# fudan-zvg/tensoflow

Measured on NVIDIA B200. Metric: train rays/sec (fwd+bwd), higher is better.
Workload: dtype f32

## Files before the change

tensoflow_b200/csrc/mlp.cu:

```cuda
#include "common.cuh"
#include "act.cuh"

namespace {

constexpr int BM = 128, BN = 64, BK = 16, BMP = BM + 4, BNP = BN + 4;

template <bool TRANS_W, bool BWD>
__global__ void __launch_bounds__(256, 2) linear_kernel(const float* __restrict__ A, int lda, const float* __restrict__ Yact,
                                                        float* __restrict__ dpre, const float* __restrict__ W, int ldw,
                                                        const float* __restrict__ bias, int64_t M, int Kred, int Nout, int act,
                                                        float act_p, float* __restrict__ out, int ldo) {
    __shared__ __align__(16) float As[BK][BMP];
    __shared__ __align__(16) float Bs[BK][BNP];
    const int64_t r0 = (int64_t)blockIdx.x * BM;
    const int c0 = blockIdx.y * BN;
    const int ty = threadIdx.x / 16, tx = threadIdx.x % 16;
    float acc[8][4];
#pragma unroll
    for (int i = 0; i < 8; ++i) acc[i][0] = acc[i][1] = acc[i][2] = acc[i][3] = 0.f;
    for (int k0 = 0; k0 < Kred; k0 += BK) {
#pragma unroll
        for (int i = 0; i < BM / 16; ++i) {
            const int row = ty + 16 * i, k = tx;
            const int64_t r = r0 + row;
// ... 222 lines not shown
int tf_internal_xty(const float* X, int ldx, const float* Y, int ldy, int64_t rows, int M, int N, float* out, int ldo,
                    cudaStream_t stream) {
    if (rows == 0 || M == 0 || N == 0) return 0;
    dim3 grid((M + XT_M - 1) / XT_M, (N + XT_N - 1) / XT_N, 1);
    const int tiles = grid.x * grid.y;
    int64_t slices = (2 * (int64_t)tf_num_sms() + tiles - 1) / tiles;
    int64_t rpc = (rows + slices - 1) / slices;
    rpc = ((rpc + XT_R - 1) / XT_R) * XT_R;
    if (rpc < 256) rpc = 256;
    grid.z = (unsigned)((rows + rpc - 1) / rpc);
    xty_kernel<<<grid, 256, 0, stream>>>(X, ldx, Y, ldy, rows, M, N, out, ldo, rpc);
    tf_count_launches(1);
    return 0;
}

int tf_internal_matmul(const float* A, int lda, const float* W, int ldw, int64_t M, int Kred, int Nout, float* out, int ldo,
                       cudaStream_t stream) {
    if (M == 0 || Nout == 0) return 0;
    dim3 grid((unsigned)((M + BM - 1) / BM), (Nout + BN - 1) / BN);
    linear_kernel<true, false><<<grid, 256, 0, stream>>>(A, lda, nullptr, nullptr, W, ldw, nullptr, M, Kred, Nout, 0, 0.f, out, ldo);
    tf_count_launches(1);
    return 0;
}

int tf_internal_colsum(const float* X, int ldx, int64_t rows, int cols, float* out, cudaStream_t stream) {
    if (rows == 0 || cols == 0) return 0;
    int gy = (int)(rows < 1184 ? rows : 1184);
    dim3 cg((cols + 127) / 128, gy);
    colsum_kernel<<<cg, 128, 0, stream>>>(X, ldx, rows, cols, out);
    tf_count_launches(1);
    return 0;
}

constexpr int HEAD_NMAX = 8, HEAD_KMAX = 256;
bool head_shape(int64_t M, int K, int N, const void* a, const void* b) {
    return M >= 4096 && N <= HEAD_NMAX && K % 4 == 0 && K > SL_MAX && K <= HEAD_KMAX && (((uintptr_t)a | (uintptr_t)b) & 15) == 0;
}

template <int CH>
__global__ void __launch_bounds__(256) head_fwd_kernel(const float* __restrict__ X, const float* __restrict__ W, const float* __restrict__ b,
                                                       int64_t M, int K, int N, int act, float act_p, float* __restrict__ Y) {
    const int lane = threadIdx.x & 31, wpb = blockDim.x >> 5;
    float4 w[HEAD_NMAX][CH];
#pragma unroll
    for (int n = 0; n < HEAD_NMAX; ++n)
#pragma unroll
        for (int c = 0; c < CH; ++c) {
            const int k = c * 128 + lane * 4;
            w[n][c] = (n < N && k < K) ? *reinterpret_cast<const float4*>(W + (size_t)n * K + k) : f4_zero();
        }
    const float bias = (b && lane < N) ? b[lane] : 0.f;
    for (int64_t m = (int64_t)blockIdx.x * wpb + (threadIdx.x >> 5); m < M; m += (int64_t)gridDim.x * wpb) {
        float4 x[CH];
#pragma unroll
        for (int c = 0; c < CH; ++c) {
            const int k = c * 128 + lane * 4;
            x[c] = k < K ? ldg4(X + (size_t)m * K + k) : f4_zero();
        }
        float mine = 0.f;
#pragma unroll
        for (int n = 0; n < HEAD_NMAX; ++n) {
            if (n >= N) break;
            float a = 0.f;
#pragma unroll
            for (int c = 0; c < CH; ++c) a += (x[c].x * w[n][c].x + x[c].y * w[n][c].y) + (x[c].z * w[n][c].z + x[c].w * w[n][c].w);
#pragma unroll
            for (int o = 16; o > 0; o >>= 1) a += __shfl_xor_sync(0xffffffffu, a, o);
            if (lane == n) mine = a;
        }
        if (lane < N) Y[(size_t)m * N + lane] = act_fwd(mine + bias, act, act_p);
    }
}

template <int CH>
__global__ void __launch_bounds__(256) head_bwd_kernel(const float* __restrict__ X, const float* __restrict__ W, const float* __restrict__ Y,
                                                       const float* __restrict__ dY, int64_t M, int K, int N, int act, float act_p,
                                                       float* __restrict__ dX, float* __restrict__ dW, float* __restrict__ db) {
    __shared__ float red[8][HEAD_NMAX][HEAD_KMAX / 2 + 4];
    const int lane = threadIdx.x & 31, warp = threadIdx.x >> 5, wpb = blockDim.x >> 5;
    float4 w[HEAD_NMAX][CH], acc[HEAD_NMAX][CH];
#pragma unroll
    for (int n = 0; n < HEAD_NMAX; ++n)
#pragma unroll
        for (int c = 0; c < CH; ++c) {
            const int k = c * 128 + lane * 4;
            w[n][c] = (n < N && k < K) ? *reinterpret_cast<const float4*>(W + (size_t)n * K + k) : f4_zero();
            acc[n][c] = f4_zero();
        }
    float accb = 0.f;
    for (int64_t m = (int64_t)blockIdx.x * wpb + warp; m < M; m += (int64_t)gridDim.x * wpb) {
        float dp = 0.f;
        if (lane < N) { const size_t o = (size_t)m * N + lane; dp = __ldg(dY + o) * act_bwd(__ldg(Y + o), act, act_p); }
        accb += dp;
        float4 x[CH], dx[CH];
#pragma unroll
        for (int c = 0; c < CH; ++c) {
            const int k = c * 128 + lane * 4;
            x[c] = k < K ? ldg4(X + (size_t)m * K + k) : f4_zero();
            dx[c] = f4_zero();
        }
#pragma unroll
        for (int n = 0; n < HEAD_NMAX; ++n) {
            if (n >= N) break;
            const float d = __shfl_sync(0xffffffffu, dp, n);
#pragma unroll
            for (int c = 0; c < CH; ++c) { dx[c] = f4_fma(d, w[n][c], dx[c]); acc[n][c] = f4_fma(d, x[c], acc[n][c]); }
        }
        if (dX) {
#pragma unroll
            for (int c = 0; c < CH; ++c) {
                const int k = c * 128 + lane * 4;
                if (k < K) *reinterpret_cast<float4*>(dX + (size_t)m * K + k) = dx[c];
            }
        }
    }
#pragma unroll
    for (int c = 0; c < CH; ++c) {
        __syncthreads();
#pragma unroll
        for (int n = 0; n < HEAD_NMAX; ++n) *reinterpret_cast<float4*>(&red[warp][n][lane * 4]) = acc[n][c];
        __syncthreads();
        for (int i = threadIdx.x; i < N * 128; i += blockDim.x) {
            const int n = i >> 7, kk = i & 127, k = c * 128 + kk;
            if (k >= K) continue;
            float sum = 0.f;
            for (int wv = 0; wv < wpb; ++wv) sum += red[wv][n][kk];
            if (dW && sum != 0.f) atomicAdd(dW + (size_t)n * K + k, sum);
        }
    }
    if (db) {
        __syncthreads();
        if (lane < N) red[warp][lane][0] = accb;
        __syncthreads();
        if (threadIdx.x < N) {
            float sum = 0.f;
            for (int wv = 0; wv < wpb; ++wv) sum += red[wv][threadIdx.x][0];
            if (sum != 0.f) atomicAdd(db + threadIdx.x, sum);
        }
    }
}

int head_grid(int64_t M) {
    const int64_t want = (M + 127) / 128, cap = (int64_t)tf_num_sms() * 4;
    return (int)(want < cap ? want : cap);
}

bool tf_internal_linear_tc_ok(const float* X, const float* Y, int K, int N, int act);
size_t tf_internal_linear_tc_ws_floats(int K, int N);
int tf_internal_linear_tc(const float* X, const float* W, int ldw, int trans, const float* bias, int64_t M, int K, int N, int act, float act_p,
                          float* Y, float* wtc, cudaStream_t stream);
int tf_internal_linear_tc_bwd(const float* dY, const float* Yact, float* dpre, const float* W, int64_t M, int K, int N, int act, float act_p,
                              float* dX, float* wtc, cudaStream_t stream);
bool tf_internal_xty_tc_ok(const float* X, const float* Y, int M, int N);
int tf_internal_xty_tc(const float* X, const float* Y, int64_t rows, int M, int N, float* out, int ldo, int n_valid, cudaStream_t stream);

static const int64_t TC_MIN_ROWS = 8192;
static bool tc_shape(int64_t M, int K, int N) { return M >= TC_MIN_ROWS && K >= 96 && N >= 96; }

extern "C" TF_API size_t tf_linear_workspace(int32_t K, int32_t N) {
    if (K < 1 || N < 1) return 0;
    const size_t a = tf_internal_linear_tc_ws_floats(K, N), b = tf_internal_linear_tc_ws_floats(N, K);
    return (a > b ? a : b) * sizeof(float);
}

extern "C" TF_API int tf_linear_fwd(const float* X, const float* W, const float* b, int64_t M, int32_t K, int32_t N, int32_t act,
                                    float act_param, float* Y, void* workspace, size_t ws_bytes, tf_stream_t stream) {
    if (M == 0) return 0;
    TF_REQUIRE(X && W && Y, "tf_linear_fwd: NULL pointer");
    TF_REQUIRE(K > 0 && N > 0 && act >= 0 && act <= 5, "tf_linear_fwd: bad K/N/act (%d,%d,%d)", K, N, act);
    if (head_shape(M, K, N, X, W)) {
        if (K <= 128) head_fwd_kernel<1><<<head_grid(M), 256, 0, (cudaStream_t)stream>>>(X, W, b, M, K, N, act, act_param, Y);
        else head_fwd_kernel<2><<<head_grid(M), 256, 0, (cudaStream_t)stream>>>(X, W, b, M, K, N, act, act_param, Y);
        tf_count_launches(1);
        TF_CHECK_LAUNCH("tf_linear_fwd (head)");
        return 0;
    }
    if (workspace && tc_shape(M, K, N) && tf_internal_linear_tc_ok(X, Y, K, N, act) && ((uintptr_t)workspace & 15) == 0 &&
        ws_bytes >= tf_internal_linear_tc_ws_floats(K, N) * sizeof(float)) {
        tf_internal_linear_tc(X, W, K, 0, b, M, K, N, act, act_param, Y, (float*)workspace, (cudaStream_t)stream);
        TF_CHECK_LAUNCH("tf_linear_fwd (tcgen05)");
        return 0;
    }
    dim3 grid((unsigned)((M + BM - 1) / BM), (N + BN - 1) / BN);
    linear_kernel<false, false><<<grid, 256, 0, (cudaStream_t)stream>>>(X, K, nullptr, nullptr, W, K, b, M, K, N, act, act_param, Y, N);
    tf_count_launches(1);
    TF_CHECK_LAUNCH("tf_linear_fwd");
    return 0;
}

extern "C" TF_API int tf_linear_bwd(const float* X, const float* W, const float* Y, const float* dY, float* dpre, int64_t M,
                                    int32_t K, int32_t N, int32_t act, float act_param, float* dX, float* dW, float* db,
                                    void* workspace, size_t ws_bytes, tf_stream_t stream_) {
    if (M == 0) return 0;
    TF_REQUIRE(X && W && Y && dY && dpre && dY != dpre, "tf_linear_bwd: NULL pointer (or dY aliases dpre)");
    TF_REQUIRE(K > 0 && N > 0 && act >= 0 && act <= 5, "tf_linear_bwd: bad K/N/act (%d,%d,%d)", K, N, act);
    cudaStream_t stream = (cudaStream_t)stream_;
    if (K <= SL_MAX && N <= SL_MAX && M >= 4096) {
        const size_t smem = sizeof(float) * ((size_t)SL_ROWS * SL_DS + (size_t)SL_ROWS * SL_XS + (size_t)SL_MAX * SL_XS);
        cudaFuncSetAttribute(small_linear_bwd_kernel, cudaFuncAttributeMaxDynamicSharedMemorySize, (int)smem);
        const int64_t ntiles = (M + SL_ROWS - 1) / SL_ROWS;
        const int grid = (int)(ntiles < 2 * tf_num_sms() ? ntiles : 2 * tf_num_sms());
        small_linear_bwd_kernel<<<grid, 256, smem, stream>>>(X, W, Y, dY, M, K, N, act, act_param, dX, dW, db);
        tf_count_launches(1);
        TF_CHECK_LAUNCH("tf_linear_bwd (narrow)");
        return 0;
    }
    if (head_shape(M, K, N, X, W) && (!dX || ((uintptr_t)dX & 15) == 0)) {
        if (K <= 128) head_bwd_kernel<1><<<head_grid(M), 256, 0, stream>>>(X, W, Y, dY, M, K, N, act, act_param, dX, dW, db);
        else head_bwd_kernel<2><<<head_grid(M), 256, 0, stream>>>(X, W, Y, dY, M, K, N, act, act_param, dX, dW, db);
        tf_count_launches(1);
        TF_CHECK_LAUNCH("tf_linear_bwd (head)");
        return 0;
    }
    if (dX && workspace && tc_shape(M, K, N) && tf_internal_linear_tc_ok(dY, dX, N, K, act) && ((uintptr_t)workspace & 15) == 0 &&
        ws_bytes >= tf_internal_linear_tc_ws_floats(N, K) * sizeof(float)) {
        tf_internal_linear_tc_bwd(dY, Y, dpre, W, M, K, N, act, act_param, dX, (float*)workspace, stream);
    } else if (dX) {
        dim3 grid((unsigned)((M + BM - 1) / BM), (K + BN - 1) / BN);
        linear_kernel<true, true><<<grid, 256, 0, stream>>>(dY, N, Y, dpre, W, K, nullptr, M, N, K, act, act_param, dX, K);
        tf_count_launches(1);
    } else {
        dim3 grid((unsigned)((M + BM - 1) / BM), 1);
        linear_kernel<true, true><<<grid, 256, 0, stream>>>(dY, N, Y, dpre, W, K, nullptr, M, N, 0, act, act_param, nullptr, K);
        tf_count_launches(1);
    }
    if (dW) {
        if (tc_shape(M, K, N) && K % 16 == 0 && tf_internal_xty_tc_ok(dpre, X, N, K)) tf_internal_xty_tc(dpre, X, M, N, K, dW, K, K, stream);
        else tf_internal_xty(dpre, N, X, K, M, N, K, dW, K, stream);
    }
    if (db) tf_internal_colsum(dpre, N, M, N, db, stream);
    TF_CHECK_LAUNCH("tf_linear_bwd");
    return 0;
}
```

tensoflow_b200/csrc/sdf_stencil.cu:

```cuda
#include <stdlib.h>
#include "common.cuh"

namespace {

constexpr int TS = 16;
constexpr int NQ = 7;
constexpr int R = TS * NQ;
constexpr int NC = 32;
constexpr int NT = 256;
constexpr int HCS = NC + 2;

__host__ __device__ inline int round_up4(int x) { return (x + 3) & ~3; }

__global__ void prep_weights_kernel(const float* __restrict__ W0, const float* __restrict__ W1, int K, int KP, int H, int A,
                                    float* __restrict__ W0T, float* __restrict__ W0P, float* __restrict__ W1T) {
    const int tid = blockIdx.x * blockDim.x + threadIdx.x, nth = gridDim.x * blockDim.x;
    for (int i = tid; i < KP * H; i += nth) {
        const int k = i / H, h = i % H;
        W0T[i] = k < K ? W0[h * K + k] : 0.f;
    }
    for (int i = tid; i < H * KP; i += nth) {
        const int h = i / KP, k = i % KP;
        W0P[i] = k < K ? W0[h * K + k] : 0.f;
    }
// ... 386 lines not shown
    TF_REQUIRE(m && m->W0 && m->b0 && m->W1 && m->b1, "MLP descriptor / weights are NULL");
    TF_REQUIRE(m->hidden > 0 && m->hidden % NC == 0, "hidden must be a multiple of %d (got %d)", NC, m->hidden);
    TF_REQUIRE(m->app_dim >= 4 && m->app_dim % 4 == 0 && m->app_dim <= 128, "app_dim must be a multiple of 4 in [4,128] (got %d)", m->app_dim);
    TF_REQUIRE(f->n_comp <= 36, "n_comp <= 36 supported by the fused stencil (got %d)", f->n_comp);
    d.C = f->n_comp; d.K = 3 * d.C + 3; d.KP = round_up4(d.K); d.KS = d.KP + 4; d.H = m->hidden; d.A = m->app_dim;
    return 0;
}

size_t weights_ws_floats(const Dims& d) { return (size_t)2 * d.KP * d.H + (size_t)d.H * d.A; }

size_t fwd_smem(const Dims& d, bool feat) {
    return sizeof(float) * ((size_t)R * d.KS + (size_t)d.KP * NC + (feat ? (size_t)NC * d.A + TS * HCS : 0));
}
size_t bwd_smem(const Dims& d) {
    return sizeof(float) * ((size_t)R * d.KS + (size_t)d.KP * NC + (size_t)NC * d.KS + (size_t)R * DSS + (size_t)TS * d.A +
                            (size_t)(1 + d.A) * NC + NQ * TS + 2 * d.H + 4);
}

void fill_common(StencilParams& p, const tf_vm_field_t* f, const tf_sdf_mlp_t* m, const Dims& d, const float* xyz,
                 const float* level, int64_t n, const float units[3], float* ws) {
    p.f = *f; p.xyz = xyz; p.level = level; p.n = n;
    p.W0T = ws; p.W0P = ws + (size_t)d.KP * d.H; p.W1T = ws + (size_t)2 * d.KP * d.H;
    p.b0 = m->b0; p.W1 = m->W1; p.b1 = m->b1;
    p.K = d.K; p.KP = d.KP; p.KS = d.KS; p.H = d.H; p.A = d.A;
    p.units[0] = units ? units[0] : 0.f; p.units[1] = units ? units[1] : 0.f; p.units[2] = units ? units[2] : 0.f;
}

}

int tf_check_field(const tf_vm_field_t* f, bool need_mips);

bool tf_internal_linear_tc_ok(const float* X, const float* Y, int K, int N, int act);
size_t tf_internal_linear_tc_ws_floats(int K, int N);
int tf_internal_linear_tc(const float* X, const float* W, int ldw, int trans, const float* bias, int64_t M, int K, int N, int act, float act_p,
                          float* Y, float* wtc, cudaStream_t stream);
size_t tf_internal_tc_fwd_smem(int KT, int H);
size_t tf_internal_tc_w0_floats(int KT, int H);
int tf_internal_stencil_fwd_tc(const tf_vm_field_t* f, const tf_sdf_mlp_t* m, const float* xyz, const float* level, int64_t n,
                               const float units[3], int nq, float* sdf7, float* grad, float* hess, float* sdf1, float* spc,
                               float* w0tc, cudaStream_t stream);
static bool use_simt_path(const Dims& d) {
    static int forced = -1;
    if (forced < 0) { const char* e = getenv("TF_STENCIL_SIMT"); forced = (e && e[0] == '1') ? 1 : 0; }
    const int KT = (d.K + 15) / 16 * 16;
    return forced == 1 || tf_internal_tc_fwd_smem(KT, d.H) > 227 * 1024 || KT > 128 || d.H > 256 || d.H % 32 != 0;
}

static size_t fwd_ws_floats(const Dims& d, int64_t n, bool with_feat) {
    if (use_simt_path(d)) return weights_ws_floats(d);
    const int KT = (d.K + 15) / 16 * 16;
    return tf_internal_tc_w0_floats(KT, d.H) + (with_feat ? (size_t)(n < 1 ? 1 : n) * d.H + tf_internal_linear_tc_ws_floats(d.H, d.A) : 0);
}

extern "C" TF_API size_t tf_sdf_stencil_fwd_workspace(const tf_vm_field_t* f, const tf_sdf_mlp_t* m, int64_t n, int32_t with_feat) {
    Dims d;
    if (!f || !m || check_mlp(f, m, d)) return 0;
    return fwd_ws_floats(d, n, with_feat != 0) * sizeof(float);
}

static int stencil_fwd_impl(int mode, const tf_vm_field_t* f, const tf_sdf_mlp_t* m, const float* xyz, const float* level,
                            int64_t n, const float units[3], float* sdf7, float* feat, float* grad, float* hess, float* sdf1,
                            void* workspace, size_t ws_bytes, tf_stream_t stream_) {
    if (int e = tf_check_field(f, level != nullptr)) return e;
    Dims d;
    if (int e = check_mlp(f, m, d)) return e;
    if (n == 0) return 0;
    TF_REQUIRE(xyz, "xyz is NULL");
    TF_REQUIRE(workspace && ws_bytes >= fwd_ws_floats(d, n, feat != nullptr) * sizeof(float), "workspace too small (%zu bytes)", ws_bytes);
    TF_REQUIRE(((uintptr_t)workspace & 15) == 0, "workspace not 16-byte aligned");
    if (feat) TF_REQUIRE(((uintptr_t)feat & 15) == 0, "feat not 16-byte aligned");
    cudaStream_t stream = (cudaStream_t)stream_;
    if (!use_simt_path(d)) {
        const int KT = (d.K + 15) / 16 * 16;
        float* w0tc = (float*)workspace;
        float* spc = feat ? w0tc + tf_internal_tc_w0_floats(KT, d.H) : nullptr;
        if (mode == 0) TF_REQUIRE(sdf7, "sdf7 is NULL"); else TF_REQUIRE(sdf1, "sdf is NULL");
        if (int e = tf_internal_stencil_fwd_tc(f, m, xyz, level, n, units, mode == 0 ? 7 : 1, sdf7, grad, hess, sdf1, spc, w0tc, stream)) return e;
        if (feat) {
            float* wlin = spc + (size_t)n * d.H;
            if (tf_internal_linear_tc_ok(spc, feat, d.H, d.A, 0))
                tf_internal_linear_tc(spc, m->W1 + d.H, d.H, 0, m->b1 + 1, n, d.H, d.A, 0, 0.f, feat, wlin, stream);
            else if (int e = tf_linear_fwd(spc, m->W1 + d.H, m->b1 + 1, n, d.H, d.A, 0, 0.f, feat, nullptr, 0, stream_)) return e;
        }
        TF_CHECK_LAUNCH("tf_sdf_stencil_fwd (tcgen05)");
        return 0;
    }
    StencilParams p = {};
    fill_common(p, f, m, d, xyz, level, n, units, (float*)workspace);
    p.sdf7 = sdf7; p.feat = feat; p.grad = grad; p.hess = hess; p.sdf1 = sdf1;
    prep_weights_kernel<<<64, 256, 0, stream>>>(m->W0, m->W1, d.K, d.KP, d.H, d.A, (float*)p.W0T, (float*)p.W0P, (float*)p.W1T);
    const int64_t per_tile = mode == 0 ? TS : R;
    const int64_t ntiles = (n + per_tile - 1) / per_tile;
    const int64_t cap = (int64_t)tf_num_sms() * 2;
    const int grid = (int)(ntiles < cap ? ntiles : cap);
    if (mode == 0) {
        TF_REQUIRE(sdf7, "sdf7 is NULL");
        const size_t smem = fwd_smem(d, feat != nullptr);
        cudaFuncSetAttribute(sdf_stencil_fwd_kernel<0>, cudaFuncAttributeMaxDynamicSharedMemorySize, (int)smem);
        sdf_stencil_fwd_kernel<0><<<grid, NT, smem, stream>>>(p);
    } else {
        TF_REQUIRE(sdf1, "sdf is NULL");
        const size_t smem = fwd_smem(d, false);
        cudaFuncSetAttribute(sdf_stencil_fwd_kernel<1>, cudaFuncAttributeMaxDynamicSharedMemorySize, (int)smem);
        sdf_stencil_fwd_kernel<1><<<grid, NT, smem, stream>>>(p);
    }
    tf_count_launches(2);
    TF_CHECK_LAUNCH("tf_sdf_stencil_fwd");
    return 0;
}

extern "C" TF_API int tf_sdf_stencil_fwd(const tf_vm_field_t* f, const tf_sdf_mlp_t* m, const float* xyz, const float* level,
                                  int64_t n, const float units[3], float* sdf7, float* feat, float* grad, float* hess,
                                  void* workspace, size_t ws_bytes, tf_stream_t stream) {
    TF_REQUIRE(units, "units is NULL");
    return stencil_fwd_impl(0, f, m, xyz, level, n, units, sdf7, feat, grad, hess, nullptr, workspace, ws_bytes, stream);
}

extern "C" TF_API int tf_sdf_only_fwd(const tf_vm_field_t* f, const tf_sdf_mlp_t* m, const float* xyz, const float* level, int64_t n,
                               float* sdf, void* workspace, size_t ws_bytes, tf_stream_t stream) {
    return stencil_fwd_impl(1, f, m, xyz, level, n, nullptr, nullptr, nullptr, nullptr, nullptr, sdf, workspace, ws_bytes, stream);
}

extern "C" TF_API int tf_sdf_point_fwd(const tf_vm_field_t* f, const tf_sdf_mlp_t* m, const float* xyz, const float* level, int64_t n,
                                       float* sdf, float* feat, void* workspace, size_t ws_bytes, tf_stream_t stream) {
    Dims d;
    if (!f || !m) { tf_set_error("tf_sdf_point_fwd: NULL descriptor"); return 1; }
    if (int e = check_mlp(f, m, d)) return e;
    TF_REQUIRE(feat, "tf_sdf_point_fwd: feat is NULL (use tf_sdf_only_fwd for the SDF alone)");
    TF_REQUIRE(!use_simt_path(d), "tf_sdf_point_fwd: only the tensor-core path evaluates single queries with features "
                                  "(hidden %% 32 == 0, hidden <= 256); use tf_sdf_stencil_fwd");
    return stencil_fwd_impl(1, f, m, xyz, level, n, nullptr, nullptr, feat, nullptr, nullptr, sdf, workspace, ws_bytes, stream);
}

static size_t bwd_slice_floats(const Dims& d, int64_t n_slice) {
    const int64_t tiles = (n_slice + TS - 1) / TS;
    return (size_t)tiles * ((size_t)R * d.H + (size_t)R * d.KP + (size_t)TS * d.H);
}

size_t tf_internal_bwd_tc_wtc_floats(int KT, int H);
size_t tf_internal_bwd_tc_smem(int KT, int H);
int tf_internal_bwd_tc_prep(const float* W0, int K, int KT, int H, float* wtc, cudaStream_t stream);
int tf_internal_bwd_tc_samples_per_tile();
int tf_internal_bwd_tc_fold(const float* tmp, int H, int K, int KT, float* dW0, float* db0, cudaStream_t stream);
int tf_internal_stencil_bwd_tc(const tf_vm_field_t* f, const tf_vm_mut_t* g, const tf_sdf_mlp_t* m, const float* wtc, const float* xyz,
                               const float* level, int64_t n, const float units[3], const float* sdf7, const float* g_sdf,
                               const float* g_grad, const float* g_hess, const float* dHc, float* dpre, float* arow, float* spc,
                               float* da_scratch, float* dW1r0, float* db1, cudaStream_t stream);
size_t tf_internal_bwd_tc_scratch_floats(int KT);
int tf_internal_xty(const float* X, int ldx, const float* Y, int ldy, int64_t rows, int M, int N, float* out, int ldo, cudaStream_t stream);
int tf_internal_colsum(const float* X, int ldx, int64_t rows, int cols, float* out, cudaStream_t stream);
int tf_internal_matmul(const float* A, int lda, const float* W, int ldw, int64_t M, int Kred, int Nout, float* out, int ldo,
                       cudaStream_t stream);
bool tf_internal_xty_tc_ok(const float* X, const float* Y, int M, int N);
int tf_internal_xty_tc(const float* X, const float* Y, int64_t rows, int M, int N, float* out, int ldo, int n_valid, cudaStream_t stream);
int tf_internal_xty_tc_tiled(const float* X, const float* Y, int64_t rows, int M, int N, float* out, int ldo, int n_valid, int x_tiled,
                             cudaStream_t stream);

static bool use_simt_bwd(const Dims& d) {
    const int KT = (d.K + 15) / 16 * 16;
    return use_simt_path(d) || d.C % 4 != 0 || KT > 128  || tf_internal_bwd_tc_smem(KT, d.H) > 227 * 1024;
}
static size_t bwd_tc_fixed_floats(const Dims& d) {
    const int KT = (d.K + 15) / 16 * 16;
    return tf_internal_bwd_tc_wtc_floats(KT, d.H) + (size_t)d.H * KT + tf_internal_linear_tc_ws_floats(d.A, d.H) +
           tf_internal_bwd_tc_scratch_floats(KT);
}
static size_t bwd_tc_tile_floats(const Dims& d) {
    const int KT = (d.K + 15) / 16 * 16, spt = tf_internal_bwd_tc_samples_per_tile();
    return (size_t)128 * (d.H + KT) + 2 * (size_t)spt * d.H;
}

extern "C" TF_API size_t tf_sdf_stencil_bwd_workspace(const tf_vm_field_t* f, const tf_sdf_mlp_t* m, int64_t n_slice) {
    Dims d;
    if (!f || !m || check_mlp(f, m, d)) return 0;
    if (n_slice < 1) n_slice = 1;
    if (!use_simt_bwd(d)) {
        const int spt = tf_internal_bwd_tc_samples_per_tile();
        return (bwd_tc_fixed_floats(d) + (size_t)((n_slice + spt - 1) / spt) * bwd_tc_tile_floats(d)) * sizeof(float);
    }
    return (weights_ws_floats(d) + bwd_slice_floats(d, n_slice)) * sizeof(float);
}

static int stencil_bwd_tc(const tf_vm_field_t* f, const tf_sdf_mlp_t* m, const Dims& d, const float* xyz, const float* level, int64_t n,
                          const float units[3], const float* sdf7, const float* g_sdf, const float* g_feat, const float* g_grad,
                          const float* g_hess, const tf_vm_mut_t* g_field, const tf_sdf_mlp_grad_t* g_mlp, float* ws, size_t ws_floats,
                          const float* hidden_c, cudaStream_t stream) {
    const int KT = (d.K + 15) / 16 * 16, H = d.H;
    const int spt = tf_internal_bwd_tc_samples_per_tile();
    const size_t fixed = bwd_tc_fixed_floats(d), per_tile = bwd_tc_tile_floats(d);
    TF_REQUIRE(ws_floats >= fixed + per_tile, "workspace too small (%zu bytes)", ws_floats * sizeof(float));
    int64_t tiles_fit = (int64_t)((ws_floats - fixed) / per_tile);
    const int64_t ntiles_all = (n + spt - 1) / spt;
    if (tiles_fit > ntiles_all) tiles_fit = ntiles_all;
    float* wtc = ws;
    float* tmp = wtc + tf_internal_bwd_tc_wtc_floats(KT, H);
    float* wlin = tmp + (size_t)H * KT;
    float* da_scratch = wlin + tf_internal_linear_tc_ws_floats(d.A, H);
    float* dpre = da_scratch + tf_internal_bwd_tc_scratch_floats(KT);
    float* arow = dpre + (size_t)tiles_fit * 128 * H;
    float* spc = arow + (size_t)tiles_fit * 128 * KT;
    float* dHc = spc + (size_t)tiles_fit * spt * H;
    tf_internal_bwd_tc_prep(m->W0, d.K, KT, H, wtc, stream);
    cudaMemsetAsync(tmp, 0, (size_t)H * KT * sizeof(float), stream);
    for (int64_t t0 = 0; t0 < ntiles_all; t0 += tiles_fit) {
        const int64_t nt = t0 + tiles_fit < ntiles_all ? tiles_fit : ntiles_all - t0;
        const int64_t s0 = t0 * spt;
        const int64_t ns = s0 + nt * spt < n ? nt * spt : n - s0;
        const float* gf = g_feat ? g_feat + s0 * d.A : nullptr;
        if (gf) {
            if (tf_internal_linear_tc_ok(gf, dHc, d.A, H, 0)) tf_internal_linear_tc(gf, m->W1 + H, H, 1, nullptr, ns, d.A, H, 0, 0.f, dHc, wlin, stream);
            else tf_internal_matmul(gf, d.A, m->W1 + H, H, ns, d.A, H, dHc, H, stream);
        }
        if (int e = tf_internal_stencil_bwd_tc(f, g_field, m, wtc, xyz + s0 * 3, level ? level + s0 : nullptr, ns, units, sdf7 + s0 * NQ,
                                               g_sdf ? g_sdf + s0 : nullptr, g_grad ? g_grad + s0 * 3 : nullptr,
                                               g_hess ? g_hess + s0 : nullptr, gf ? dHc : nullptr, dpre, arow, (gf && !hidden_c) ? spc : nullptr,
                                               da_scratch, g_mlp->W1, g_mlp->b1, stream))
            return e;
        TF_REQUIRE(tf_internal_xty_tc_ok(dpre, arow, H, KT), "tensor-core X^T Y does not take this decoder shape (H=%d, KT=%d)", H, KT);
        if (int e = tf_internal_xty_tc_tiled(dpre, arow, nt * 128, H, KT, tmp, KT, d.K + 1, 1, stream)) return e;
        if (gf) {
            const float* hid = hidden_c ? hidden_c + s0 * H : spc;
            if (tf_internal_xty_tc_ok(gf, hid, d.A, H)) tf_internal_xty_tc(gf, hid, ns, d.A, H, g_mlp->W1 + H, H, H, stream);
            else tf_internal_xty(gf, d.A, hid, H, ns, d.A, H, g_mlp->W1 + H, H, stream);
            tf_internal_colsum(gf, d.A, ns, d.A, g_mlp->b1 + 1, stream);
        }
    }
    tf_internal_bwd_tc_fold(tmp, H, d.K, KT, g_mlp->W0, g_mlp->b0, stream);
    TF_CHECK_LAUNCH("tf_sdf_stencil_bwd (tcgen05)");
    return 0;
}

extern "C" TF_API size_t tf_sdf_stencil_fwd_hidden_offset(const tf_vm_field_t* f, const tf_sdf_mlp_t* m) {
    Dims d;
    if (!f || !m || check_mlp(f, m, d) || use_simt_path(d)) return (size_t)-1;
    const int KT = (d.K + 15) / 16 * 16;
    return tf_internal_tc_w0_floats(KT, d.H) * sizeof(float);
}

extern "C" TF_API int tf_sdf_stencil_bwd(const tf_vm_field_t* f, const tf_sdf_mlp_t* m, const float* xyz, const float* level,
                                  int64_t n, const float units[3], const float* sdf7, const float* g_sdf, const float* g_feat,
                                  const float* g_grad, const float* g_hess, const tf_vm_mut_t* g_field,
                                  const tf_sdf_mlp_grad_t* g_mlp, void* workspace, size_t ws_bytes, tf_stream_t stream_) {
    return tf_sdf_stencil_bwd_kept(f, m, xyz, level, n, units, sdf7, nullptr, g_sdf, g_feat, g_grad, g_hess, g_field, g_mlp, workspace, ws_bytes,
                                   stream_);
}

extern "C" TF_API int tf_sdf_stencil_bwd_kept(const tf_vm_field_t* f, const tf_sdf_mlp_t* m, const float* xyz, const float* level,
                                       int64_t n, const float units[3], const float* sdf7, const float* hidden_centre, const float* g_sdf,
                                       const float* g_feat, const float* g_grad, const float* g_hess, const tf_vm_mut_t* g_field,
                                       const tf_sdf_mlp_grad_t* g_mlp, void* workspace, size_t ws_bytes, tf_stream_t stream_) {
    if (int e = tf_check_field(f, level != nullptr)) return e;
    Dims d;
    if (int e = check_mlp(f, m, d)) return e;
    if (n == 0) return 0;
    TF_REQUIRE(xyz && units && sdf7, "xyz/units/sdf7 is NULL");
    TF_REQUIRE(g_field && g_mlp && g_mlp->W0 && g_mlp->b0 && g_mlp->W1 && g_mlp->b1, "gradient descriptors are NULL");
    for (int i = 0; i < 3; ++i) {
        TF_REQUIRE(g_field->plane[i] && g_field->line[i], "gradient buffer %d is NULL", i);
        if (f->n_levels > 1 && level) TF_REQUIRE(g_field->plane_mip[i] && g_field->line_mip[i], "mip gradient buffer %d is NULL", i);
    }
    TF_REQUIRE(((uintptr_t)workspace & 15) == 0, "workspace not 16-byte aligned");
    if (g_feat) TF_REQUIRE(((uintptr_t)g_feat & 15) == 0, "g_feat not 16-byte aligned");
    cudaStream_t stream = (cudaStream_t)stream_;
    float* ws = (float*)workspace;
    TF_REQUIRE(workspace, "workspace is NULL");
    if (hidden_centre) TF_REQUIRE(((uintptr_t)hidden_centre & 15) == 0, "hidden_centre not 16-byte aligned");
    if (!use_simt_bwd(d))
        return stencil_bwd_tc(f, m, d, xyz, level, n, units, sdf7, g_sdf, g_feat, g_grad, g_hess, g_field, g_mlp, ws,
                              ws_bytes / sizeof(float), hidden_centre, stream);
    const size_t wfl = weights_ws_floats(d);
    TF_REQUIRE(ws_bytes >= (wfl + bwd_slice_floats(d, TS)) * sizeof(float), "workspace too small (%zu bytes)", ws_bytes);
    const size_t per_tile = (size_t)R * d.H + (size_t)R * d.KP + (size_t)TS * d.H;
    int64_t tiles_fit = (int64_t)((ws_bytes / sizeof(float) - wfl) / per_tile);
    const int64_t ntiles_all = (n + TS - 1) / TS;
    if (tiles_fit > ntiles_all) tiles_fit = ntiles_all;
    const size_t smem = bwd_smem(d);
    cudaFuncSetAttribute(sdf_stencil_bwd_kernel, cudaFuncAttributeMaxDynamicSharedMemorySize, (int)smem);
    StencilParams p = {};
    fill_common(p, f, m, d, xyz, level, n, units, ws);
    prep_weights_kernel<<<64, 256, 0, stream>>>(m->W0, m->W1, d.K, d.KP, d.H, d.A, (float*)p.W0T, (float*)p.W0P, (float*)p.W1T);
    tf_count_launches(1);
    float* dpre = ws + wfl;
    float* arow = dpre + (size_t)tiles_fit * R * d.H;
    float* spc = arow + (size_t)tiles_fit * R * d.KP;
    for (int64_t t0 = 0; t0 < ntiles_all; t0 += tiles_fit) {
        const int64_t nt = t0 + tiles_fit < ntiles_all ? tiles_fit : ntiles_all - t0;
        const int64_t s0 = t0 * TS;
        const int64_t ns = (s0 + nt * TS < n ? nt * TS : n - s0);
        StencilParams q = p;
        q.xyz = xyz + s0 * 3; q.level = level ? level + s0 : nullptr; q.n = ns;
        q.sdf7_in = sdf7 + s0 * NQ;
        q.g_sdf = g_sdf ? g_sdf + s0 : nullptr; q.g_feat = g_feat ? g_feat + s0 * d.A : nullptr;
        q.g_grad = g_grad ? g_grad + s0 * 3 : nullptr; q.g_hess = g_hess ? g_hess + s0 : nullptr;
        q.g = *g_field;
        q.dpre = dpre; q.arow = arow; q.spc = spc;
        q.db0 = g_mlp->b0; q.dW1r0 = g_mlp->W1; q.db1 = g_mlp->b1;
        const int64_t cap = tf_num_sms();
        const int grid = (int)(nt < cap ? nt : cap);
        sdf_stencil_bwd_kernel<<<grid, NT, smem, stream>>>(q);
        tf_count_launches(1);
        tf_internal_xty(dpre, d.H, arow, d.KP, nt * R, d.H, d.K, g_mlp->W0, d.K, stream);
        if (g_feat) {
            tf_internal_xty(q.g_feat, d.A, spc, d.H, ns, d.A, d.H, g_mlp->W1 + d.H, d.H, stream);
            tf_internal_colsum(q.g_feat, d.A, ns, d.A, g_mlp->b1 + 1, stream);
        }
    }
    TF_CHECK_LAUNCH("tf_sdf_stencil_bwd");
    return 0;
}
```

tensoflow_b200/csrc/xty_tc.cu:

```cuda
#include <stdlib.h>
#include "common.cuh"
#include "tc_common.cuh"

namespace {

constexpr int NTH = 512;
constexpr int NWORK = NTH - 32;
constexpr int TPT = 2;
constexpr uint32_t LBO = 144;
template <int RS> struct Stage { static constexpr uint32_t SBO = (RS / 4) * LBO + 16; };

__device__ __forceinline__ float4 hi4(float4 v) { return make_float4(tc::tf32_rn(v.x), tc::tf32_rn(v.y), tc::tf32_rn(v.z), tc::tf32_rn(v.w)); }
__device__ __forceinline__ float4 lo4(float4 v, float4 h) {
    return make_float4(tc::tf32_rn(v.x - h.x), tc::tf32_rn(v.y - h.y), tc::tf32_rn(v.z - h.z), tc::tf32_rn(v.w - h.w));
}

struct Prefetch { float4 v[TPT][4]; };
struct StagePlan { int src_off[TPT]; int row[TPT]; int ld[TPT]; uint32_t smem_off[TPT]; bool on[TPT], is_x[TPT], tiled[TPT]; };

template <int RS>
__device__ __forceinline__ StagePlan make_stage_plan(int M, int N, int wtid, bool x_tiled, bool y_tiled) {
    constexpr uint32_t SBO = Stage<RS>::SBO;
    StagePlan p;
    const int ty = (RS / 4) * (N / 4), tx = (RS / 4) * (M / 4);
#pragma unroll
    for (int k = 0; k < TPT; ++k) {
        int it = wtid + k * NWORK;
        p.is_x[k] = it >= ty;
        if (p.is_x[k]) it -= ty;
        const int W = p.is_x[k] ? M : N, G = W / 4;
        p.on[k] = wtid >= 0 && it < (p.is_x[k] ? tx : ty);
        p.tiled[k] = p.is_x[k] ? x_tiled : y_tiled;
        const int g = p.tiled[k] ? it / (RS / 4) : it % G, c = p.tiled[k] ? it % (RS / 4) : it / G;
        p.row[k] = c * 4;
        p.ld[k] = p.tiled[k] ? 128 : W;
        p.src_off[k] = p.tiled[k] ? g * 4 * 128 + c * 4 : c * 4 * W + g * 4;
        const int w = g * 4;
        p.smem_off[k] = (uint32_t)(w >> 3) * SBO + c * LBO + (w & 7) * 16;
    }
    return p;
}
__device__ __forceinline__ void stage_load(const float* __restrict__ X, const float* __restrict__ Y, int64_t r0, int64_t r_end, int M, int N,
                                           const StagePlan& sp, Prefetch& pf) {
#pragma unroll
    for (int k = 0; k < TPT; ++k) {
        if (sp.tiled[k]) {
            const float* base = (sp.is_x[k] ? X + (size_t)(r0 >> 7) * 128 * M : Y + (size_t)(r0 >> 7) * 128 * N) + (r0 & 127) + sp.src_off[k];
#pragma unroll
            for (int i = 0; i < 4; ++i) pf.v[k][i] = (sp.on[k] && r0 + sp.row[k] < r_end) ? ldg4(base + i * 128) : make_float4(0.f, 0.f, 0.f, 0.f);
        } else {
            const float* base = (sp.is_x[k] ? X : Y) + (size_t)r0 * sp.ld[k] + sp.src_off[k];
#pragma unroll
            for (int i = 0; i < 4; ++i)
                pf.v[k][i] = (sp.on[k] && r0 + sp.row[k] + i < r_end) ? ldg4(base + i * sp.ld[k]) : make_float4(0.f, 0.f, 0.f, 0.f);
        }
    }
}
__device__ __forceinline__ void stage_store(const Prefetch& pf, const StagePlan& sp, uint8_t* xs_hi, uint8_t* xs_lo, uint8_t* ys_hi, uint8_t* ys_lo) {
#pragma unroll
    for (int k = 0; k < TPT; ++k) {
        if (!sp.on[k]) continue;
        uint8_t* hi = sp.is_x[k] ? xs_hi : ys_hi;
        uint8_t* lo = sp.is_x[k] ? xs_lo : ys_lo;
        const float4* v = pf.v[k];
        float4 t[4];
        if (sp.tiled[k]) {
            t[0] = v[0]; t[1] = v[1]; t[2] = v[2]; t[3] = v[3];
        } else {
            t[0] = make_float4(v[0].x, v[1].x, v[2].x, v[3].x); t[1] = make_float4(v[0].y, v[1].y, v[2].y, v[3].y);
            t[2] = make_float4(v[0].z, v[1].z, v[2].z, v[3].z); t[3] = make_float4(v[0].w, v[1].w, v[2].w, v[3].w);
        }
#pragma unroll
        for (int j = 0; j < 4; ++j) {
            const uint32_t off = sp.smem_off[k] + j * 16;
            const float4 h = hi4(t[j]);
            *reinterpret_cast<float4*>(hi + off) = h;
            *reinterpret_cast<float4*>(lo + off) = lo4(t[j], h);
        }
    }
}

template <int RS>
__global__ void __launch_bounds__(NTH, 1) xty_tc_kernel(const float* __restrict__ X, const float* __restrict__ Y, int64_t rows, int M, int MP, int N,
                                                        float* __restrict__ out, int ldo, int x_valid, int y_valid, int tr, int64_t rows_per_cta,
                                                        int x_tiled, int y_tiled) {
    extern __shared__ __align__(1024) uint8_t smem[];
    constexpr uint32_t SBO = Stage<RS>::SBO;
    const uint32_t x_part = (uint32_t)(MP / 8) * SBO, y_part = (uint32_t)(N / 8) * SBO;
    const uint32_t stage_bytes = 2 * (x_part + y_part);
    uint64_t* bars = reinterpret_cast<uint64_t*>(smem + 2 * stage_bytes);
    uint64_t* empty = bars;
    uint64_t* ready = bars + 2;
    uint64_t* done = bars + 4;
    uint32_t* tmem_slot = reinterpret_cast<uint32_t*>(bars + 5);
    const int tid = threadIdx.x, warp = tid >> 5, lane = tid & 31;
    const int MT = MP / 128;
    const int ncol_tile = N <= 128 ? 128 : 256;

    if (warp == 0) tc::tmem_alloc<512>(tmem_slot);
    if (tid == 0) {
        tc::mbar_init(&empty[0], 1); tc::mbar_init(&empty[1], 1); tc::mbar_init(&ready[0], NWORK); tc::mbar_init(&ready[1], NWORK);
        tc::mbar_init(done, 1);
        tc::mbar_fence_init();
    }
    for (uint32_t i = tid * 16; i < 2 * stage_bytes; i += NTH * 16) *reinterpret_cast<float4*>(smem + i) = make_float4(0.f, 0.f, 0.f, 0.f);
    tc::fence_async_smem();
    tc::fence_before_sync();
    __syncthreads();
    tc::fence_after_sync();
    const uint32_t tmem_base = *tmem_slot;
    const uint32_t idesc = tc::make_idesc(2, 2, 128, N);

    const int64_t r_begin = (int64_t)blockIdx.x * rows_per_cta;
    const int64_t r_end = r_begin + rows_per_cta < rows ? r_begin + rows_per_cta : rows;
    const int64_t n_stages = r_begin < r_end ? (r_end - r_begin + RS - 1) / RS : 0;

    if (warp == 0) {
        if (lane == 0) {
            for (int64_t it = 0; it < n_stages; ++it) {
                const int buf = (int)(it & 1);
                uint8_t* xs_hi = smem + (size_t)buf * stage_bytes;
                uint8_t* xs_lo = xs_hi + x_part;
                uint8_t* ys_hi = xs_lo + x_part;
                uint8_t* ys_lo = ys_hi + y_part;
                tc::mbar_wait(&ready[buf], (uint32_t)((it >> 1) & 1));
                tc::fence_after_sync();
                const uint64_t xdh = tc::make_smem_desc(tc::smem_u32(xs_hi), LBO, SBO), xdl = tc::make_smem_desc(tc::smem_u32(xs_lo), LBO, SBO);
                const uint64_t ydh = tc::make_smem_desc(tc::smem_u32(ys_hi), LBO, SBO), ydl = tc::make_smem_desc(tc::smem_u32(ys_lo), LBO, SBO);
#pragma unroll
                for (int ks = 0; ks < RS / 8; ++ks) {
                    const uint64_t bdh = tc::desc_add(ydh, ks * 2 * LBO), bdl = tc::desc_add(ydl, ks * 2 * LBO);
#pragma unroll
                    for (int mt = 0; mt < 2; ++mt) {
                        if (mt >= MT) break;
                        const uint32_t d = tmem_base + (uint32_t)mt * ncol_tile;
                        const uint64_t adh = tc::desc_add(xdh, mt * 16 * SBO + ks * 2 * LBO), adl = tc::desc_add(xdl, mt * 16 * SBO + ks * 2 * LBO);
                        tc::mma_tf32_ss(d, adh, bdh, idesc, (it | ks) != 0);
                        tc::mma_tf32_ss(d, adh, bdl, idesc, 1);
                        tc::mma_tf32_ss(d, adl, bdh, idesc, 1);
                    }
                }
                tc::mma_commit(&empty[buf]);
                if (it == n_stages - 1) tc::mma_commit(done);
            }
        }
    } else {
        Prefetch p0, p1;
        const StagePlan sp = make_stage_plan<RS>(M, N, tid - 32, x_tiled != 0, y_tiled != 0);
        if (n_stages > 0) stage_load(X, Y, r_begin, r_end, M, N, sp, p0);
        if (n_stages > 1) stage_load(X, Y, r_begin + RS, r_end, M, N, sp, p1);
        auto do_stage = [&](int64_t it, Prefetch& pf) {
            const int buf = (int)(it & 1);
            uint8_t* xs_hi = smem + (size_t)buf * stage_bytes;
            uint8_t* xs_lo = xs_hi + x_part;
            uint8_t* ys_hi = xs_lo + x_part;
            uint8_t* ys_lo = ys_hi + y_part;
            if (it >= 2) tc::mbar_wait(&empty[buf], (uint32_t)(((it >> 1) - 1) & 1));
            stage_store(pf, sp, xs_hi, xs_lo, ys_hi, ys_lo);
            if (it + 2 < n_stages) stage_load(X, Y, r_begin + (it + 2) * RS, r_end, M, N, sp, pf);
            tc::fence_async_smem();
            tc::mbar_arrive(&ready[buf]);
        };
        for (int64_t it = 0; it < n_stages; it += 2) {
            do_stage(it, p0);
            if (it + 1 < n_stages) do_stage(it + 1, p1);
        }
    }
    __syncwarp();
    if (n_stages > 0) {
        tc::mbar_wait(done, 0);
        tc::fence_after_sync();
        const int lq = warp & 3, half = warp >> 2;
        for (int mt = 0; mt < MT; ++mt) {
            const int m = mt * 128 + lq * 32 + lane;
            for (int c0 = half * 16; c0 < N; c0 += 16 * (NTH / 128)) {
                float v[16];
                tc::tmem_ld16(tmem_base + (uint32_t)mt * ncol_tile + ((uint32_t)(lq * 32) << 16) + c0, v);
#pragma unroll
                for (int j = 0; j < 16; ++j)
                    if (m < x_valid && c0 + j < y_valid && v[j] != 0.f)
                        atomicAdd(tr ? out + (size_t)(c0 + j) * ldo + m : out + (size_t)m * ldo + c0 + j, v[j]);
            }
        }
    }
    tc::fence_before_sync();
    __syncthreads();
    if (warp == 0) tc::tmem_dealloc<512>(tmem_base);
}

size_t xty_tc_smem(int MP, int N, int rs) { return (size_t)2 * 2 * ((MP / 8) + (N / 8)) * ((rs / 4) * LBO + 16) + 64; }
int xty_tc_stage_rows(int MP, int N) { return xty_tc_smem(MP, N, 32) <= 227 * 1024 ? 32 : 16; }

}

bool tf_internal_xty_tc_ok(const float* X, const float* Y, int M, int N) {
    if (M % 16 != 0 || N % 16 != 0 || M < 16 || N < 16 || M > 256 || N > 256) return false;
    if (((uintptr_t)X & 15) || ((uintptr_t)Y & 15)) return false;
    const int mw = M > N ? N : M, nw = M > N ? M : N;
    return xty_tc_smem((mw + 127) / 128 * 128, nw, 16) <= 227 * 1024;
}

int tf_internal_xty_tc_tiled(const float* X, const float* Y, int64_t rows, int M, int N, float* out, int ldo, int n_valid, int x_tiled,
                             cudaStream_t stream);
int tf_internal_xty_tc(const float* X, const float* Y, int64_t rows, int M, int N, float* out, int ldo, int n_valid, cudaStream_t stream) {
    return tf_internal_xty_tc_tiled(X, Y, rows, M, N, out, ldo, n_valid, 0, stream);
}
int tf_internal_xty_tc_tiled(const float* X, const float* Y, int64_t rows, int M, int N, float* out, int ldo, int n_valid, int x_tiled,
                             cudaStream_t stream) {
    if (rows == 0) return 0;
    const bool tr = M > N;
    const float* xs = tr ? Y : X;
    const float* ys = tr ? X : Y;
    const int mw = tr ? N : M, nw = tr ? M : N;
    const int mp = (mw + 127) / 128 * 128;
    const int x_valid = tr ? n_valid : M, y_valid = tr ? M : n_valid;
    const int RS = xty_tc_stage_rows(mp, nw);
    const size_t smem = xty_tc_smem(mp, nw, RS);
    int64_t grid = (rows + 4 * RS - 1) / (4 * RS);
    if (grid > tf_num_sms()) grid = tf_num_sms();
    int64_t rpc = (rows + grid - 1) / grid;
    const int64_t rgran = x_tiled ? 128 : RS;
    rpc = (rpc + rgran - 1) / rgran * rgran;
    grid = (rows + rpc - 1) / rpc;
    if (x_tiled && rows % 128 != 0) { tf_set_error("xty_tc: a tiled operand needs rows to be a multiple of 128"); return 1; }
    const int kx_tiled = (x_tiled && !tr) ? 1 : 0, ky_tiled = (x_tiled && tr) ? 1 : 0;
    {
        TfKernelTimer timer("xty_tc", stream);
        if (RS == 32) {
            cudaFuncSetAttribute(xty_tc_kernel<32>, cudaFuncAttributeMaxDynamicSharedMemorySize, (int)smem);
            xty_tc_kernel<32><<<(int)grid, NTH, smem, stream>>>(xs, ys, rows, mw, mp, nw, out, ldo, x_valid, y_valid, tr ? 1 : 0, rpc, kx_tiled, ky_tiled);
        } else {
            cudaFuncSetAttribute(xty_tc_kernel<16>, cudaFuncAttributeMaxDynamicSharedMemorySize, (int)smem);
            xty_tc_kernel<16><<<(int)grid, NTH, smem, stream>>>(xs, ys, rows, mw, mp, nw, out, ldo, x_valid, y_valid, tr ? 1 : 0, rpc, kx_tiled, ky_tiled);
        }
    }
    tf_count_launches(1);
    return 0;
}

int tf_internal_xty(const float* X, int ldx, const float* Y, int ldy, int64_t rows, int M, int N, float* out, int ldo, cudaStream_t stream);

extern "C" TF_API int tf_xty_accumulate(const float* X, const float* Y, int64_t rows, int32_t M, int32_t N, float* out,
                                        int32_t force_simt, tf_stream_t stream_) {
    if (rows == 0) return 0;
    TF_REQUIRE(X && Y && out && M > 0 && N > 0, "tf_xty_accumulate: NULL pointer or bad shape (%d,%d)", M, N);
    cudaStream_t stream = (cudaStream_t)stream_;
    if (!force_simt && tf_internal_xty_tc_ok(X, Y, M, N)) tf_internal_xty_tc(X, Y, rows, M, N, out, N, N, stream);
    else tf_internal_xty(X, M, Y, N, rows, M, N, out, N, stream);
    TF_CHECK_LAUNCH("tf_xty_accumulate");
    return 0;
}
```

Before: 85080.

## Fuse bias-gradient column sum into tensor-core X^T Y weight-gradient kernel

Adds an optional fused column-sum to the tcgen05 X^T Y kernel: loader threads accumulate per-column sums of the staged gradient operand in registers, reduce them through shared memory, then atomically add into the bias gradient. Linear backward and the appearance-head weight gradient in the stencil backward use this instead of a separate colsum launch. With cached hidden activations, the appearance weight-gradient is also hoisted out of the per-slice loop into one full-batch call. This saves a launch and a second read of dpre, at the cost of extra register pressure, 1KB more shared memory, and float atomics that make the summation order nondeterministic.

```diff
diff --git a/tensoflow_b200/csrc/mlp.cu b/tensoflow_b200/csrc/mlp.cu
--- a/tensoflow_b200/csrc/mlp.cu
+++ b/tensoflow_b200/csrc/mlp.cu
@@ -398,7 +398,8 @@
 int tf_internal_linear_tc_bwd(const float* dY, const float* Yact, float* dpre, const float* W, int64_t M, int K, int N, int act, float act_p,
                               float* dX, float* wtc, cudaStream_t stream);
 bool tf_internal_xty_tc_ok(const float* X, const float* Y, int M, int N);
-int tf_internal_xty_tc(const float* X, const float* Y, int64_t rows, int M, int N, float* out, int ldo, int n_valid, cudaStream_t stream);
+int tf_internal_xty_tc(const float* X, const float* Y, int64_t rows, int M, int N, float* out, int ldo, int n_valid, float* colsum,
+                       cudaStream_t stream);
 
 static const int64_t TC_MIN_ROWS = 8192;
 static bool tc_shape(int64_t M, int K, int N) { return M >= TC_MIN_ROWS && K >= 96 && N >= 96; }
@@ -470,11 +471,12 @@
         linear_kernel<true, true><<<grid, 256, 0, stream>>>(dY, N, Y, dpre, W, K, nullptr, M, N, 0, act, act_param, nullptr, K);
         tf_count_launches(1);
     }
-    if (dW) {
-        if (tc_shape(M, K, N) && K % 16 == 0 && tf_internal_xty_tc_ok(dpre, X, N, K)) tf_internal_xty_tc(dpre, X, M, N, K, dW, K, K, stream);
-        else tf_internal_xty(dpre, N, X, K, M, N, K, dW, K, stream);
-    }
-    if (db) tf_internal_colsum(dpre, N, M, N, db, stream);
+    if (dW && tc_shape(M, K, N) && K % 16 == 0 && tf_internal_xty_tc_ok(dpre, X, N, K)) {
+        tf_internal_xty_tc(dpre, X, M, N, K, dW, K, K, db, stream);
+    } else {
+        if (dW) tf_internal_xty(dpre, N, X, K, M, N, K, dW, K, stream);
+        if (db) tf_internal_colsum(dpre, N, M, N, db, stream);
+    }
     TF_CHECK_LAUNCH("tf_linear_bwd");
     return 0;
 }
diff --git a/tensoflow_b200/csrc/sdf_stencil.cu b/tensoflow_b200/csrc/sdf_stencil.cu
--- a/tensoflow_b200/csrc/sdf_stencil.cu
+++ b/tensoflow_b200/csrc/sdf_stencil.cu
@@ -562,9 +562,10 @@
 int tf_internal_matmul(const float* A, int lda, const float* W, int ldw, int64_t M, int Kred, int Nout, float* out, int ldo,
                        cudaStream_t stream);
 bool tf_internal_xty_tc_ok(const float* X, const float* Y, int M, int N);
-int tf_internal_xty_tc(const float* X, const float* Y, int64_t rows, int M, int N, float* out, int ldo, int n_valid, cudaStream_t stream);
+int tf_internal_xty_tc(const float* X, const float* Y, int64_t rows, int M, int N, float* out, int ldo, int n_valid, float* colsum,
+                       cudaStream_t stream);
 int tf_internal_xty_tc_tiled(const float* X, const float* Y, int64_t rows, int M, int N, float* out, int ldo, int n_valid, int x_tiled,
-                             cudaStream_t stream);
+                             float* colsum, cudaStream_t stream);
 
 static bool use_simt_bwd(const Dims& d) {
     const int KT = (d.K + 15) / 16 * 16;
@@ -589,6 +590,17 @@
         return (bwd_tc_fixed_floats(d) + (size_t)((n_slice + spt - 1) / spt) * bwd_tc_tile_floats(d)) * sizeof(float);
     }
     return (weights_ws_floats(d) + bwd_slice_floats(d, n_slice)) * sizeof(float);
+}
+
+static void appearance_wgrad(const float* gf, const float* hid, int64_t rows, const Dims& d, const tf_sdf_mlp_grad_t* g_mlp,
+                             cudaStream_t stream) {
+    const int H = d.H;
+    if (tf_internal_xty_tc_ok(gf, hid, d.A, H)) {
+        tf_internal_xty_tc(gf, hid, rows, d.A, H, g_mlp->W1 + H, H, H, g_mlp->b1 + 1, stream);
+    } else {
+        tf_internal_xty(gf, d.A, hid, H, rows, d.A, H, g_mlp->W1 + H, H, stream);
+        tf_internal_colsum(gf, d.A, rows, d.A, g_mlp->b1 + 1, stream);
+    }
 }
 
 static int stencil_bwd_tc(const tf_vm_field_t* f, const tf_sdf_mlp_t* m, const Dims& d, const float* xyz, const float* level, int64_t n,
@@ -627,14 +639,10 @@
                                                da_scratch, g_mlp->W1, g_mlp->b1, stream))
             return e;
         TF_REQUIRE(tf_internal_xty_tc_ok(dpre, arow, H, KT), "tensor-core X^T Y does not take this decoder shape (H=%d, KT=%d)", H, KT);
-        if (int e = tf_internal_xty_tc_tiled(dpre, arow, nt * 128, H, KT, tmp, KT, d.K + 1, 1, stream)) return e;
-        if (gf) {
-            const float* hid = hidden_c ? hidden_c + s0 * H : spc;
-            if (tf_internal_xty_tc_ok(gf, hid, d.A, H)) tf_internal_xty_tc(gf, hid, ns, d.A, H, g_mlp->W1 + H, H, H, stream);
-            else tf_internal_xty(gf, d.A, hid, H, ns, d.A, H, g_mlp->W1 + H, H, stream);
-            tf_internal_colsum(gf, d.A, ns, d.A, g_mlp->b1 + 1, stream);
-        }
-    }
+        if (int e = tf_internal_xty_tc_tiled(dpre, arow, nt * 128, H, KT, tmp, KT, d.K + 1, 1, nullptr, stream)) return e;
+        if (gf && !hidden_c) appearance_wgrad(gf, spc, ns, d, g_mlp, stream);
+    }
+    if (g_feat && hidden_c) appearance_wgrad(g_feat, hidden_c, n, d, g_mlp, stream);
     tf_internal_bwd_tc_fold(tmp, H, d.K, KT, g_mlp->W0, g_mlp->b0, stream);
     TF_CHECK_LAUNCH("tf_sdf_stencil_bwd (tcgen05)");
     return 0;
diff --git a/tensoflow_b200/csrc/xty_tc.cu b/tensoflow_b200/csrc/xty_tc.cu
--- a/tensoflow_b200/csrc/xty_tc.cu
+++ b/tensoflow_b200/csrc/xty_tc.cu
@@ -16,7 +16,7 @@
 }
 
 struct Prefetch { float4 v[TPT][4]; };
-struct StagePlan { int src_off[TPT]; int row[TPT]; int ld[TPT]; uint32_t smem_off[TPT]; bool on[TPT], is_x[TPT], tiled[TPT]; };
+struct StagePlan { int src_off[TPT]; int row[TPT]; int ld[TPT]; int col[TPT]; uint32_t smem_off[TPT]; bool on[TPT], is_x[TPT], tiled[TPT]; };
 
 template <int RS>
 __device__ __forceinline__ StagePlan make_stage_plan(int M, int N, int wtid, bool x_tiled, bool y_tiled) {
@@ -36,6 +36,7 @@
         p.ld[k] = p.tiled[k] ? 128 : W;
         p.src_off[k] = p.tiled[k] ? g * 4 * 128 + c * 4 : c * 4 * W + g * 4;
         const int w = g * 4;
+        p.col[k] = w;
         p.smem_off[k] = (uint32_t)(w >> 3) * SBO + c * LBO + (w & 7) * 16;
     }
     return p;
@@ -80,10 +81,10 @@
     }
 }
 
-template <int RS>
+template <int RS, bool CS>
 __global__ void __launch_bounds__(NTH, 1) xty_tc_kernel(const float* __restrict__ X, const float* __restrict__ Y, int64_t rows, int M, int MP, int N,
                                                         float* __restrict__ out, int ldo, int x_valid, int y_valid, int tr, int64_t rows_per_cta,
-                                                        int x_tiled, int y_tiled) {
+                                                        int x_tiled, int y_tiled, float* __restrict__ csum, int cs_x) {
     extern __shared__ __align__(1024) uint8_t smem[];
     constexpr uint32_t SBO = Stage<RS>::SBO;
     const uint32_t x_part = (uint32_t)(MP / 8) * SBO, y_part = (uint32_t)(N / 8) * SBO;
@@ -93,6 +94,7 @@
     uint64_t* ready = bars + 2;
     uint64_t* done = bars + 4;
     uint32_t* tmem_slot = reinterpret_cast<uint32_t*>(bars + 5);
+    float* cs_smem = reinterpret_cast<float*>(smem + 2 * stage_bytes + 64);
     const int tid = threadIdx.x, warp = tid >> 5, lane = tid & 31;
     const int MT = MP / 128;
     const int ncol_tile = N <= 128 ? 128 : 256;
@@ -104,6 +106,7 @@
         tc::mbar_fence_init();
     }
     for (uint32_t i = tid * 16; i < 2 * stage_bytes; i += NTH * 16) *reinterpret_cast<float4*>(smem + i) = make_float4(0.f, 0.f, 0.f, 0.f);
+    if (CS && tid < 256) cs_smem[tid] = 0.f;
     tc::fence_async_smem();
     tc::fence_before_sync();
     __syncthreads();
@@ -147,6 +150,9 @@
     } else {
         Prefetch p0, p1;
         const StagePlan sp = make_stage_plan<RS>(M, N, tid - 32, x_tiled != 0, y_tiled != 0);
+        float4 cs[TPT];
+#pragma unroll
+        for (int k = 0; k < TPT; ++k) cs[k] = make_float4(0.f, 0.f, 0.f, 0.f);
         if (n_stages > 0) stage_load(X, Y, r_begin, r_end, M, N, sp, p0);
         if (n_stages > 1) stage_load(X, Y, r_begin + RS, r_end, M, N, sp, p1);
         auto do_stage = [&](int64_t it, Prefetch& pf) {
@@ -156,6 +162,16 @@
             uint8_t* ys_hi = xs_lo + x_part;
             uint8_t* ys_lo = ys_hi + y_part;
             if (it >= 2) tc::mbar_wait(&empty[buf], (uint32_t)(((it >> 1) - 1) & 1));
+            if (CS) {
+#pragma unroll
+                for (int k = 0; k < TPT; ++k) {
+                    const float4* v = pf.v[k];
+                    if (sp.on[k] && sp.is_x[k] == (cs_x != 0)) {
+                        cs[k].x += (v[0].x + v[1].x) + (v[2].x + v[3].x); cs[k].y += (v[0].y + v[1].y) + (v[2].y + v[3].y);
+                        cs[k].z += (v[0].z + v[1].z) + (v[2].z + v[3].z); cs[k].w += (v[0].w + v[1].w) + (v[2].w + v[3].w);
+                    }
+                }
+            }
             stage_store(pf, sp, xs_hi, xs_lo, ys_hi, ys_lo);
             if (it + 2 < n_stages) stage_load(X, Y, r_begin + (it + 2) * RS, r_end, M, N, sp, pf);
             tc::fence_async_smem();
@@ -164,6 +180,14 @@
         for (int64_t it = 0; it < n_stages; it += 2) {
             do_stage(it, p0);
             if (it + 1 < n_stages) do_stage(it + 1, p1);
+        }
+        if (CS) {
+#pragma unroll
+            for (int k = 0; k < TPT; ++k)
+                if (sp.on[k] && sp.is_x[k] == (cs_x != 0)) {
+                    float* c = cs_smem + sp.col[k];
+                    atomicAdd(c, cs[k].x); atomicAdd(c + 1, cs[k].y); atomicAdd(c + 2, cs[k].z); atomicAdd(c + 3, cs[k].w);
+                }
         }
     }
     __syncwarp();
@@ -186,9 +210,14 @@
     tc::fence_before_sync();
     __syncthreads();
     if (warp == 0) tc::tmem_dealloc<512>(tmem_base);
-}
-
-size_t xty_tc_smem(int MP, int N, int rs) { return (size_t)2 * 2 * ((MP / 8) + (N / 8)) * ((rs / 4) * LBO + 16) + 64; }
+    if (CS) {
+        const int w = cs_x ? M : N;
+        for (int c = tid; c < w; c += NTH)
+            if (cs_smem[c] != 0.f) atomicAdd(csum + c, cs_smem[c]);
+    }
+}
+
+size_t xty_tc_smem(int MP, int N, int rs) { return (size_t)2 * 2 * ((MP / 8) + (N / 8)) * ((rs / 4) * LBO + 16) + 64 + 1024; }
 int xty_tc_stage_rows(int MP, int N) { return xty_tc_smem(MP, N, 32) <= 227 * 1024 ? 32 : 16; }
 
 }
@@ -201,13 +230,15 @@
 }
 
 int tf_internal_xty_tc_tiled(const float* X, const float* Y, int64_t rows, int M, int N, float* out, int ldo, int n_valid, int x_tiled,
-                             cudaStream_t stream);
-int tf_internal_xty_tc(const float* X, const float* Y, int64_t rows, int M, int N, float* out, int ldo, int n_valid, cudaStream_t stream) {
-    return tf_internal_xty_tc_tiled(X, Y, rows, M, N, out, ldo, n_valid, 0, stream);
+                             float* colsum, cudaStream_t stream);
+int tf_internal_xty_tc(const float* X, const float* Y, int64_t rows, int M, int N, float* out, int ldo, int n_valid, float* colsum,
+                       cudaStream_t stream) {
+    return tf_internal_xty_tc_tiled(X, Y, rows, M, N, out, ldo, n_valid, 0, colsum, stream);
 }
 int tf_internal_xty_tc_tiled(const float* X, const float* Y, int64_t rows, int M, int N, float* out, int ldo, int n_valid, int x_tiled,
-                             cudaStream_t stream) {
+                             float* colsum, cudaStream_t stream) {
     if (rows == 0) return 0;
+    if (x_tiled && colsum) { tf_set_error("xty_tc: the fused column sum takes a row-major operand only"); return 1; }
     const bool tr = M > N;
     const float* xs = tr ? Y : X;
     const float* ys = tr ? X : Y;
@@ -224,15 +255,15 @@
     grid = (rows + rpc - 1) / rpc;
     if (x_tiled && rows % 128 != 0) { tf_set_error("xty_tc: a tiled operand needs rows to be a multiple of 128"); return 1; }
     const int kx_tiled = (x_tiled && !tr) ? 1 : 0, ky_tiled = (x_tiled && tr) ? 1 : 0;
+    const int cs_x = tr ? 0 : 1;
+    auto launch = [&](auto kernel) {
+        cudaFuncSetAttribute(kernel, cudaFuncAttributeMaxDynamicSharedMemorySize, (int)smem);
+        kernel<<<(int)grid, NTH, smem, stream>>>(xs, ys, rows, mw, mp, nw, out, ldo, x_valid, y_valid, tr ? 1 : 0, rpc, kx_tiled, ky_tiled, colsum, cs_x);
+    };
     {
         TfKernelTimer timer("xty_tc", stream);
-        if (RS == 32) {
-            cudaFuncSetAttribute(xty_tc_kernel<32>, cudaFuncAttributeMaxDynamicSharedMemorySize, (int)smem);
-            xty_tc_kernel<32><<<(int)grid, NTH, smem, stream>>>(xs, ys, rows, mw, mp, nw, out, ldo, x_valid, y_valid, tr ? 1 : 0, rpc, kx_tiled, ky_tiled);
-        } else {
-            cudaFuncSetAttribute(xty_tc_kernel<16>, cudaFuncAttributeMaxDynamicSharedMemorySize, (int)smem);
-            xty_tc_kernel<16><<<(int)grid, NTH, smem, stream>>>(xs, ys, rows, mw, mp, nw, out, ldo, x_valid, y_valid, tr ? 1 : 0, rpc, kx_tiled, ky_tiled);
-        }
+        if (RS == 32) colsum ? launch(xty_tc_kernel<32, true>) : launch(xty_tc_kernel<32, false>);
+        else colsum ? launch(xty_tc_kernel<16, true>) : launch(xty_tc_kernel<16, false>);
     }
     tf_count_launches(1);
     return 0;
@@ -245,7 +276,7 @@
     if (rows == 0) return 0;
     TF_REQUIRE(X && Y && out && M > 0 && N > 0, "tf_xty_accumulate: NULL pointer or bad shape (%d,%d)", M, N);
     cudaStream_t stream = (cudaStream_t)stream_;
-    if (!force_simt && tf_internal_xty_tc_ok(X, Y, M, N)) tf_internal_xty_tc(X, Y, rows, M, N, out, N, N, stream);
+    if (!force_simt && tf_internal_xty_tc_ok(X, Y, M, N)) tf_internal_xty_tc(X, Y, rows, M, N, out, N, N, nullptr, stream);
     else tf_internal_xty(X, M, Y, N, rows, M, N, out, N, stream);
     TF_CHECK_LAUNCH("tf_xty_accumulate");
     return 0;
```

After: 86000, median of 6. 1.01x the previous value.
